# rsutormin/KmerGutsJava

Hardware: AMD Instinct MI355X
Metric: amino-acid residues/sec scanned (and hits/sec) on 1 Gbp synthetic, 1/2/4/8 MI355X (higher is better)
Workload: dtype int64; 1 GPU; 1 Gbp contig mix (0.5 kbp..1.024 Mbp, uniform ACGT) on 1 GPU, 6-frame translate + 8-mer lookup vs 1400303159-slot signature table (33.6 GB, load 0.50), -m 5 -g 200; total_bp_rank0=1000000000, contigs_rank0=6351, total_bp_all_ranks=1000000000, num_sigs=1400303159, residues_rank0=1999974596, residues_all_ranks=1999974596, hits_rank0=36744843, hits_all_ranks=36744843, calls_rank0=4, parallelism=contig shards x1, table replicated

## Files before the change

kmergutsjava_amd/csrc/kg_host_plan.hpp:

```cpp
#pragma once

namespace {


template <typename T, T V, T... Vs, typename F>
void dispatch(T x, F &&f)
{
    if constexpr (sizeof...(Vs) == 0) f(std::integral_constant<T, V>{});
    else if (x == V) f(std::integral_constant<T, V>{});
    else dispatch<T, Vs...>(x, f);
}

struct BatchPlan {
    std::vector<uint32_t> ibase;
    uint64_t nblocks = 0, windows = 0, residues = 0;
    uint64_t n_rows = 0, n_cont = 0;
    int64_t longest = 0;
};

template <bool AA>
int plan_batch(const int64_t *offsets, int64_t n_seqs, BatchPlan &b)
{
    constexpr uint32_t PER = AA ? 1 : 6;
    b.ibase.resize((size_t)n_seqs + 1);
    for (int64_t k = 0; k < n_seqs; k++) {
        int64_t L = offsets[k + 1] - offsets[k];
        if (L < 0) return fail(KG_ERR_ARG, "offsets must be non-decreasing");
        b.longest = std::max(b.longest, L);
        if (L > 0xFFFFFFF0ll) return fail(KG_ERR_LIMIT, "a single sequence longer than 2^32-16 characters");
        b.ibase[(size_t)k] = (uint32_t)b.nblocks;
        uint64_t nb;
        if (AA) {
            uint64_t nwin = L >= 9 ? (uint64_t)L - 8 : 0;
            b.windows += nwin;
            b.residues += (uint64_t)L;
            nb = (nwin + kg::kAaWinPerBlock - 1) / kg::kAaWinPerBlock;
        } else {
            uint64_t npos = L >= 24 ? (uint64_t)L - 23 : 0;
            b.windows += 2 * npos;
            for (int f = 0; f < 3; f++)
                if (L - f >= 3) b.residues += 2 * (uint64_t)((L - f) / 3);
            nb = (npos + kg::kDnaPosPerBlock - 1) / kg::kDnaPosPerBlock;
        }
        b.nblocks += nb;
        if (b.nblocks > 0x7FFFFFFFull / PER) return fail(KG_ERR_LIMIT, "batch too large: more than 2^31-1 window rows; split the batch");
    }
    b.ibase[(size_t)n_seqs] = (uint32_t)b.nblocks;
    if (b.windows > 0xFFFFFF00ull) return fail(KG_ERR_LIMIT, "batch too large: more than 2^32-256 windows; split the batch");
    b.n_rows = b.nblocks * PER;
    b.n_cont = (uint64_t)n_seqs * PER;
    return KG_OK;
}

uint64_t bucket_count(uint64_t limit, uint32_t shift) { return (limit + (1ull << shift) - 1) >> shift; }

struct PartPlan {
    bool applicable = false;
    uint32_t shift = 0, buckets = 0;
    uint32_t n_chunks = 0;
    std::vector<uint64_t> clo;
    std::vector<int64_t> cseq;
    uint64_t max_chunk = 0;
    uint32_t n_wg = 0, cap = 0;
    uint64_t n_regions = 0;
    uint32_t ovf_cap = 0;
    uint32_t gshift = 10, groups_stride = 0;
    size_t next_stride = 0;
    size_t scatter_lds = 0;
    bool use_bidx = false, part_counters = false, prog_index = false;
    uint32_t probe_grid = 0, index_grid = 0, verify_grid = 0, lowc_grid = 0, ovf_grid = 0, order_grid = 0;
    uint32_t scatter_prio = 0, index_prio = 0, verify_prio = 0, index_r = 1, probe_grab = 0;
    uint32_t flush_list = 0;
    uint64_t list_slack = 0, ucap = 0, ccap = 0;
    uint32_t n_os = 0;
    bool early_totals = false, place_staged = false, debug = false;
};

template <bool AA>
int plan_partition(const kg_table *t, const BatchPlan &b, bool progress, bool counters_req, PartPlan &pl)
{
    constexpr uint32_t PER = AA ? 1 : 6;
    const uint64_t nblocks = b.nblocks;
    uint32_t shift = env_knob("KG_PART_SHIFT", 21u, 4u, 31u);
    const uint64_t qmax = (uint64_t)KG_MAX_ENCODED / (uint64_t)t->num_sigs + 1;
    while (shift > 4 && qmax >= (1ull << (32 - shift))) shift--;
    while (bucket_count(t->limit, shift) > (uint64_t)kg::kMaxBuckets) shift++;
    while (kg::scatter_lds_bytes<AA>((uint32_t)bucket_count(t->limit, shift)) > 160u * 1024) shift++;
    const bool fits = shift < 32 && qmax < (1ull << (32 - shift)) && nblocks <= (1ull << 23) && t->m35 != 0 &&
                      t->limit < (1ull << 32) - 64;
    const uint32_t mode = env_u32("KG_PARTITION", 2u);
    const bool worth = t->limit >= (64ull << 20) && b.windows >= (1ull << 27);
    if (!(fits && nblocks > 0 && (mode == 1 || (mode == 2 && worth)))) return KG_OK;
    pl.shift = shift;
    pl.buckets = (uint32_t)bucket_count(t->limit, shift);

    constexpr uint32_t WIN = AA ? 64u : 384u;
    uint32_t want = env_u32("KG_PART_CHUNKS", 4u);
    if (want < 1) want = 1;
    if (want > kMaxChunks) want = kMaxChunks;
    if (getenv("KG_PART_MIN_CHUNK_BLOCKS")) {
        const uint64_t min_chunk = std::max(1u, env_u32("KG_PART_MIN_CHUNK_BLOCKS", 600000u));
        while (want > 1 && nblocks / want < min_chunk) want--;
    } else {
        const uint32_t by_size = nblocks < 450000 ? 1u : std::max(2u, (uint32_t)std::lround(std::sqrt((double)nblocks / 325000.0)));
        want = std::min(want, std::max(1u, by_size));
    }
    pl.clo.push_back(0); pl.cseq.push_back(0);
    std::vector<double> cum;
    if (const char *tp = getenv("KG_PART_TAPER")) {
        double acc = 0;
        for (const char *q = tp; *q;) {
            char *endp = nullptr;
            const double v = strtod(q, &endp);
            if (endp == q) break;
            acc += v; cum.push_back(acc);
            q = *endp == ',' ? endp + 1 : endp;
        }
        if (cum.size() >= 2 && cum.size() <= kMaxChunks && acc > 0) { for (auto &x : cum) x /= acc; want = (uint32_t)cum.size(); }
        else cum.clear();
    }
    for (uint32_t c = 1; c < want; c++) {
        const uint64_t target = cum.empty() ? nblocks * c / want : (uint64_t)((double)nblocks * cum[c - 1]);
        const auto it = std::lower_bound(b.ibase.begin(), b.ibase.end(), (uint32_t)target);
        const uint64_t cut = *it;
        if (cut > pl.clo.back() && cut < nblocks) { pl.clo.push_back(cut); pl.cseq.push_back((int64_t)(it - b.ibase.begin())); }
    }
    pl.clo.push_back(nblocks); pl.cseq.push_back((int64_t)b.ibase.size() - 1);
    pl.n_chunks = (uint32_t)pl.clo.size() - 1;
    for (uint32_t c = 0; c < pl.n_chunks; c++) pl.max_chunk = std::max(pl.max_chunk, pl.clo[c + 1] - pl.clo[c]);
    const uint64_t max_chunk = pl.max_chunk;
    const uint64_t chunk_blocks = (max_chunk + kg::kScatterWaves - 1) / kg::kScatterWaves * kg::kScatterWaves;
    const double max_frac = (double)max_chunk / (double)nblocks;
    uint32_t n_wg = env_knob("KG_PART_WGS", 256u, 1u, kMaxGrid);
    if ((uint64_t)n_wg * kg::kScatterWaves > chunk_blocks) n_wg = (uint32_t)((chunk_blocks + kg::kScatterWaves - 1) / kg::kScatterWaves);
    const uint64_t blocks_per_wg = ((chunk_blocks + (uint64_t)n_wg * kg::kScatterWaves - 1) / ((uint64_t)n_wg * kg::kScatterWaves)) * kg::kScatterWaves;
    const double mean = (double)blocks_per_wg * WIN / (double)pl.buckets * (env_u32("KG_PART_SLACK", 100u) / 100.0);
    const uint64_t cap64 = ((uint64_t)(mean + 6.0 * std::sqrt(mean) + 32.0) + 15) / 16 * 16;
    if (cap64 >= (1ull << 24) || (uint64_t)pl.buckets * n_wg >= (1ull << 24)) return KG_OK;
    pl.n_wg = n_wg;
    pl.cap = (uint32_t)cap64;
    pl.n_regions = (uint64_t)pl.buckets * n_wg;
    pl.ovf_cap = env_u32("KG_PART_OVF_GROUPS", (uint32_t)std::min<uint64_t>(1u << 23, std::max<uint64_t>(65536, pl.n_regions * pl.cap / 16 / 8)));
    while (pl.gshift < 12 && ((max_chunk * PER) >> pl.gshift) + 2 > 8192) pl.gshift++;
    pl.groups_stride = (uint32_t)(((max_chunk * PER) >> pl.gshift) + 2);
    if (pl.groups_stride > kg::kMaxGroups) return fail(KG_ERR_LIMIT, "a chunk of the batch holds more than 2^26 window rows");
    pl.next_stride = std::max<size_t>((size_t)pl.buckets + 8, 256);
    pl.use_bidx = t->d_bidx != nullptr && !counters_req && env_u32("KG_BIDX", 1u) != 0;
    pl.part_counters = (counters_req || progress) && !pl.use_bidx;
    pl.prog_index = progress && pl.use_bidx;
    pl.scatter_lds = kg::scatter_lds_bytes<AA>(pl.buckets);
    pl.flush_list = env_knob("KG_SCATTER_FLUSH_LIST", kg::scatter_flush_list_max<AA>(), 1u, kg::scatter_flush_list_max<AA>());
    pl.probe_grid = env_knob("KG_PROBE_GRID", 256u * 8u, 8u, kMaxGrid, 8u);
    pl.index_grid = env_knob("KG_INDEX_GRID", 256u * 4u, 8u, kMaxGrid, 8u);
    pl.scatter_prio = std::min(3u, env_u32("KG_SCATTER_PRIO", 1u));
    pl.index_prio = std::min(3u, env_u32("KG_INDEX_PRIO", 2u));
    pl.verify_prio = std::min(3u, env_u32("KG_VERIFY_PRIO", pl.n_chunks == 1 ? 2u : 0u));
    uint32_t index_r = env_u32("KG_INDEX_R", 0u);
    if (index_r == 0) index_r = mean * 0.7 >= 640.0 ? 1u : mean * 0.7 >= 320.0 ? 2u : 4u;
    if (index_r != 1 && index_r != 2) index_r = 4;
    while (index_r > 1 && (n_wg % index_r != 0 || kg::kIndexN % index_r != 0)) index_r /= 2;
    pl.index_r = index_r;
    pl.verify_grid = env_knob("KG_VERIFY_GRID", 256u * 2u, 1u, kMaxGrid);
    pl.lowc_grid = env_knob("KG_LOWC_GRID", 256u, 1u, kMaxGrid);
    pl.ovf_grid = env_knob("KG_OVF_GRID", 256u, 1u, kMaxGrid);
    pl.list_slack = (uint64_t)(std::max(std::max(pl.probe_grid, pl.index_grid), pl.verify_grid) + 64) * 4 * kg::kUChunk + 4096;
    pl.ucap = ((uint64_t)((double)b.windows * t->stage_ratio * max_frac) + pl.list_slack + kg::kUChunk - 1) / kg::kUChunk * kg::kUChunk;
    pl.ccap = ((uint64_t)((double)b.windows * (t->stage_ratio * 1.25 + 0.03) * max_frac) + pl.list_slack + kg::kUChunk - 1) /
              kg::kUChunk * kg::kUChunk;
    if (test_hook("KG_TEST_TINY_LISTS")) pl.ucap = pl.ccap = kg::kUChunk;
    const uint32_t grab_unit = 256u * (uint32_t)std::max(kg::kProbeN, kg::kIndexN);
    pl.probe_grab = env_knob("KG_PROBE_GRAB", pl.cap, grab_unit, 1u << 24, grab_unit);
    pl.n_os = pl.n_chunks < 2 ? 0u : std::min(env_u32("KG_ORDER_STREAMS", 0u), kMaxOrderStreams);
    pl.early_totals = pl.n_os == 0 && env_u32("KG_EARLY_TOTALS", 1u) != 0;
    pl.order_grid = env_knob("KG_ORDER_GRID", 256u * 3u, 1u, kMaxGrid);
    pl.place_staged = pl.gshift == 10 && env_u32("KG_PLACE_STAGED", 1u) != 0;
    pl.debug = getenv("KG_DEBUG") != nullptr;
    pl.applicable = true;
    return KG_OK;
}

struct DirectPlan {
    uint32_t scan_grid, stage_chunk;
    const uint32_t *d_hbits;
    uint32_t rpg;
    uint64_t stage_cap;
};

template <bool AA>
DirectPlan plan_direct(const kg_table *t, const BatchPlan &b, bool counters)
{
    DirectPlan pl;
    pl.scan_grid = env_knob("KG_SCAN_GRID", 256u * 8u, 1u, kMaxGrid);
    pl.stage_chunk = env_knob("KG_STAGE_CHUNK", 256u, 1u, 1u << 12);
    const uint32_t filter_mode = env_u32("KG_DIRECT_FILTER", 1u);
    pl.d_hbits = (counters || filter_mode == 0 || (filter_mode == 1 && t->limit <= (4ull << 20))) ? nullptr : t->d_hbits;
    pl.rpg = AA ? 1u : env_u32("KG_SCAN_RPG", pl.d_hbits ? 6u : 3u);
    if (pl.rpg != 1 && pl.rpg != 2 && pl.rpg != 3 && pl.rpg != 6) pl.rpg = 3;
    pl.stage_cap = (uint64_t)((double)b.windows * t->stage_ratio) + 4096 + (uint64_t)pl.scan_grid * kg::kWavesPerWG * pl.stage_chunk;
    if (pl.stage_cap > 0xFFFFFF00ull) pl.stage_cap = 0xFFFFFF00ull;
    if (test_hook("KG_TEST_TINY_LISTS")) pl.stage_cap = 256;
    return pl;
}

struct AggPlan {
    uint32_t pshift;
    bool pieces_on;
    uint32_t agg_pairs;
};

AggPlan plan_aggregate()
{
    AggPlan pl;
    pl.pshift = std::min(20u, std::max(6u, env_u32("KG_AGG_BLOCK_SHIFT", 9u)));
    pl.pieces_on = env_u32("KG_AGG_PIECES", 1u) != 0;
    pl.agg_pairs = env_u32("KG_AGG_PAIRS", 1u);
    return pl;
}

}
```

kmergutsjava_amd/csrc/kg_host_scan.hpp:

```cpp
#pragma once

namespace {

struct ScanCtx {
    kg_table *t;
    kg_result *res;
    Scratch &sc;
    const BatchPlan &b;
    const uint8_t *d_seq, *h_seq;
    const int64_t *offsets;
    int64_t n_seqs;
    bool progress, counters;
    bool seq_uploaded;
    uint64_t n_hits = 0;
    int64_t *d_off = nullptr;
    uint32_t *d_ibase = nullptr;
    kg::BlockDesc *d_blocks = nullptr;
    uint32_t *d_counts = nullptr, *d_offs = nullptr, *d_bsb = nullptr;
    uint64_t *d_partial = nullptr, *d_totals = nullptr;
    kg::Progress *d_prog = nullptr;
};

int upload_seq(const ScanCtx &cx, int64_t a, int64_t b)
{
// ... 220 lines not shown
            hipLaunchKernelGGL((kg::bucket_tag_kernel<COUNTERS>), dim3(pl.probe_grid), dim3(256), 0, s2, t->d_tags, t->limit,
                               (uint64_t)t->num_sigs, v.ent, v.fill, pl.n_wg, pl.cap, pl.buckets, pl.shift, pl.probe_grab, v.next, v.cand,
                               v.candused, v.ccur, pb.ccap, d_ctr, COUNTERS ? d_prog : (kg::Progress *)nullptr);
        });
    }
    HIP_TRY(hipEventRecord(t->pev[kPevChunk + 2 * v.c + 1], s2));
    HIP_TRY(hipStreamWaitEvent(s3, t->pev[kPevChunk + 2 * v.c + 1], 0));
    dispatch<int, 1, 2, 0>(pl.part_counters ? 1 : pl.prog_index ? 2 : 0, [&](auto walks) {
        constexpr bool COUNTERS = decltype(walks)::value == 1, PROG = decltype(walks)::value == 2;
        hipLaunchKernelGGL((kg::verify_kernel<AA, COUNTERS, PROG>), dim3(pl.verify_grid), dim3(256), 0, s3, t->d_entries, t->d_tags, t->limit,
                           (uint64_t)t->num_sigs, t->magic, v.cand, v.candused, v.ccur, pb.ccap, v.ulist, v.cused, v.ucur, pb.ucap, d_ctr,
                           d_prog, pl.verify_prio);
        hipLaunchKernelGGL((kg::overflow_probe_kernel<AA, COUNTERS, PROG>), dim3(pl.ovf_grid), dim3(256), 0, s3, t->d_entries, t->d_tags,
                           t->limit, (uint64_t)t->num_sigs, t->magic, v.ovf_bucket, v.ovf_ent, v.ovfc, pl.ovf_cap, pl.shift, v.ulist,
                           v.cused, v.ucur, pb.ucap, d_ctr, d_prog);
    });
    HIP_TRY(hipEventRecord(t->pev[kPevVerified + v.c], s3));
    HIP_TRY(hipGetLastError());
    return KG_OK;
}

template <bool AA>
int chunk_order(const ScanCtx &cx, const PartPlan &pl, const PartBuffers &pb, const ChunkView &v, uint64_t hits_cap)
{
    constexpr uint32_t PER = AA ? 1 : 6;
    kg_table *t = cx.t;
    kg_result *res = cx.res;
    const uint32_t c = v.c, gshift = pl.gshift;
    const bool last = c + 1 == pl.n_chunks;
    hipStream_t s = t->stream;
    if (pl.n_os) {
        s = t->ostream[c % pl.n_os];
        HIP_TRY(hipStreamWaitEvent(s, t->ev[kEvScattered], 0));
    }
    HIP_TRY(hipStreamWaitEvent(s, t->pev[kPevVerified + c], 0));
    const uint64_t row_lo = (uint64_t)v.lo * PER, row_hi = row_lo + (uint64_t)v.nb * PER;
    const uint32_t g0 = (uint32_t)(row_lo >> gshift);
    const uint32_t n_groups = v.nb ? (uint32_t)(((row_hi - 1) >> gshift) - g0 + 1) : 1u;
    hipLaunchKernelGGL(kg::hit_hist_kernel, dim3(pl.order_grid), dim3(kg::kHThreads), (size_t)n_groups * 4, s, v.ulist, v.cused, v.ucur, pb.ucap,
                       g0, 6u + gshift, n_groups, v.ghist);
    hipLaunchKernelGGL(kg::group_scan_kernel, dim3(1), dim3(kg::kGsThreads), 0, s, v.ghist, n_groups, v.gbase, v.gcur1, v.gcur2, v.ctot, v.gtile);
    if (pl.n_os && c) HIP_TRY(hipStreamWaitEvent(s, t->pev[kPevBase + c - 1], 0));
    hipLaunchKernelGGL(kg::chunk_base_kernel, dim3(1), dim3(1), 0, s, v.ctot, v.base, last ? cx.d_totals : (uint64_t *)nullptr);
    if (pl.n_os) HIP_TRY(hipEventRecord(t->pev[kPevBase + c], s));
    if (pl.early_totals && last) {
        int rc;
        if ((rc = send_counters(t, pb.d_pc, pb.d_ovfc, cx.d_totals, s))) return rc;
        HIP_TRY(hipEventRecord(t->pev[kPevTotals], s));
    }
    hipLaunchKernelGGL((kg::hit_partition_kernel<true>), dim3(pl.order_grid), dim3(kg::kHThreads), 0, s, v.ulist, v.cused, v.ucur, pb.ucap,
                       v.gbase, n_groups, g0, 6u + gshift, v.gcur1, v.sortA, pb.ucap, v.gtile);
    hipLaunchKernelGGL((kg::hit_partition_kernel<false>), dim3(pl.order_grid), dim3(kg::kHThreads), 0, s, v.sortA, v.cused, v.ucur, pb.ucap,
                       v.gbase, n_groups, g0, 6u + gshift, v.gcur2, v.sortB, pb.ucap, v.gtile);
    hipLaunchKernelGGL((kg::group_place_kernel<AA>), dim3(std::min(n_groups, 256u * 8u)), dim3(kg::kHThreads),
                       kg::group_place_lds(gshift, pl.place_staged), s,
                       v.sortB, v.gbase, n_groups, g0, gshift, (uint32_t)row_lo, (uint32_t)row_hi, pb.d_geo, (uint64_t)cx.b.n_rows,
                       pl.place_staged ? 1u : 0u, v.base, res->d_hits, hits_cap, cx.d_offs, res->d_hit_slots);
    HIP_TRY(hipGetLastError());
    return KG_OK;
}

template <bool AA>
int part_allocate(ScanCtx &cx, const PartPlan &pl, PartBuffers &pb)
{
    kg_table *t = cx.t;
    Scratch &sc = cx.sc;
    const uint32_t n_chunks = pl.n_chunks, groups_stride = pl.groups_stride;
    int rc;
    if ((rc = sc.get(&pb.d_ent, (size_t)(pl.n_regions * pl.cap * n_chunks)))) return rc;
    if ((rc = sc.get(&pb.d_fill, (size_t)pl.n_regions * n_chunks))) return rc;
    if ((rc = sc.get(&pb.d_ovf_ent, (size_t)pl.ovf_cap * kg::kGroup * n_chunks))) return rc;
    if ((rc = sc.get(&pb.d_ovf_bucket, (size_t)pl.ovf_cap * n_chunks))) return rc;
    if ((rc = sc.get(&pb.d_next, pl.next_stride * n_chunks))) return rc;
    if ((rc = sc.get(&pb.d_ovfc, kOvfWords * kMaxChunks))) return rc;
    if ((rc = sc.get(&pb.d_lowc, (size_t)cx.b.nblocks + 1))) return rc;
    if ((rc = sc.get(&pb.d_geo, (size_t)cx.b.n_rows))) return rc;
    if ((rc = sc.get(&pb.d_ghist, (size_t)groups_stride * n_chunks))) return rc;
    if ((rc = sc.get(&pb.d_gbase, (size_t)(groups_stride + 1) * n_chunks))) return rc;
    if ((rc = sc.get(&pb.d_gcur1, (size_t)(kg::kHDigits + 1) * n_chunks))) return rc;
    if ((rc = sc.get(&pb.d_gcur2, (size_t)groups_stride * n_chunks))) return rc;
    if ((rc = sc.get(&pb.d_gtile, (size_t)(kg::kHDigits + 1) * n_chunks))) return rc;
    if (kg::group_place_lds(pl.gshift, pl.gshift == 10) > t->place_lds[AA ? 1 : 0]) {
        const size_t want_lds = kg::group_place_lds(pl.gshift, pl.gshift == 10);
        HIP_TRY(hipFuncSetAttribute((const void *)kg::group_place_kernel<AA>, hipFuncAttributeMaxDynamicSharedMemorySize, (int)want_lds));
        t->place_lds[AA ? 1 : 0] = want_lds;
    }
    if (groups_stride * 4u > t->hist_lds) {
        HIP_TRY(hipFuncSetAttribute((const void *)kg::hit_hist_kernel, hipFuncAttributeMaxDynamicSharedMemorySize, (int)(groups_stride * 4u)));
        t->hist_lds = groups_stride * 4u;
    }
    if ((rc = sc.get(&pb.d_pc, kPcWords))) return rc;
    const int sv = scatter_variant_of(cx);
    if (t->scatter_lds[AA ? 1 : 0][sv] < pl.scatter_lds) {
        hipError_t e = hipSuccess;
        scatter_variant(sv, [&](auto is_short, auto prog) {
            e = hipFuncSetAttribute((const void *)kg::part_scatter_kernel<AA, decltype(is_short)::value, decltype(prog)::value>,
                                    hipFuncAttributeMaxDynamicSharedMemorySize, (int)pl.scatter_lds);
        });
        HIP_TRY(e);
        t->scatter_lds[AA ? 1 : 0][sv] = pl.scatter_lds;
    }
    return KG_OK;
}

template <bool AA>
int scan_partitioned(ScanCtx &cx, const PartPlan &pl, bool &done)
{
    constexpr uint32_t PER = AA ? 1 : 6;
    kg_table *t = cx.t;
    kg_result *res = cx.res;
    kg_stats &st = res->st;
    const uint32_t n_chunks = pl.n_chunks;
    const uint64_t nblocks = cx.b.nblocks;
    int rc;
    PartBuffers pb;
    if ((rc = part_allocate<AA>(cx, pl, pb))) return rc;
    BlockGuard<6> lists{cx.sc, {(void **)&pb.d_ulist, (void **)&pb.d_cused, (void **)&pb.d_cand, (void **)&pb.d_candused,
                                (void **)&pb.d_sortA, (void **)&pb.d_sortB}};
    pb.ucap = pl.ucap; pb.ccap = pl.ccap;
    HIP_TRY(hipEventRecord(t->ev[kEvScanBegin], t->stream));
    for (int attempt = 0; attempt < 3; attempt++) {
        const uint64_t ucap = pb.ucap, ccap = pb.ccap;
        const uint64_t hits_cap = ucap * n_chunks;
        pb.cused_stride = (size_t)(ucap / kg::kUChunk + 1); pb.candused_stride = (size_t)(ccap / kg::kUChunk + 1);
        if ((rc = dalloc(t, (void **)&res->d_hits, hits_cap * sizeof(kg_hit)))) return rc;
        if (cx.progress && (rc = dalloc(t, (void **)&res->d_hit_slots, hits_cap * 4))) return rc;
        if ((rc = dalloc(t, (void **)&pb.d_ulist, ucap * n_chunks * sizeof(kg_hit)))) return rc;
        if ((rc = dalloc(t, (void **)&pb.d_cused, pb.cused_stride * n_chunks * 4))) return rc;
        if ((rc = dalloc(t, (void **)&pb.d_cand, ccap * n_chunks * sizeof(kg::CandRec)))) return rc;
        if ((rc = dalloc(t, (void **)&pb.d_candused, pb.candused_stride * n_chunks * 4))) return rc;
        if ((rc = dalloc(t, (void **)&pb.d_sortA, ucap * n_chunks * sizeof(kg_hit)))) return rc;
        if ((rc = dalloc(t, (void **)&pb.d_sortB, ucap * n_chunks * sizeof(kg_hit)))) return rc;
        if ((rc = clear_words(t->stream, [](uint64_t most) { return (uint32_t)std::min<uint64_t>(4096, (most / 4 + 255) / 256 + 1); },
                              {{pb.d_cused, (uint64_t)pb.cused_stride * n_chunks},
                               {pb.d_candused, (uint64_t)pb.candused_stride * n_chunks},
                               {pb.d_pc, kPcWords * 2},
                               {cx.d_totals, kTotWords * 2},
// ... 270 lines not shown
```

kmergutsjava_amd/csrc/kg_order.hpp:

```cpp
#pragma once

#include "kg_device.hpp"
#include "kg_partition.hpp"

namespace kg {

constexpr uint32_t kHThreads = 512;
constexpr uint32_t kHPer = 4;
constexpr uint32_t kHTile = kHThreads * kHPer;
constexpr uint32_t kHDigits = 128;
constexpr uint32_t kMaxGroups = kHDigits * kHDigits;

struct RowGeo { uint32_t container; int32_t pos_first; };

template <bool AA>
__global__ void row_geo_kernel(const BlockDesc *__restrict__ blocks, uint32_t n_blocks, RowGeo *__restrict__ geo)
{
    constexpr uint32_t ROWS = AA ? 1 : 6;
    const uint64_t tl = (uint64_t)blockIdx.x * blockDim.x + threadIdx.x;
    if (tl >= (uint64_t)n_blocks * ROWS) return;
    const uint32_t r = (uint32_t)(tl / n_blocks), it = (uint32_t)(tl % n_blocks);
    const BlockDesc bd = blocks[it];
    RowGeo g;
    int32_t pos0;
// ... 44 lines not shown
        }
        uint32_t incl = mine;
        for (int off = 1; off < 64; off <<= 1) {
            const uint32_t y = __shfl_up(incl, off);
            if (lane >= off) incl += y;
        }
        if (lane == 63) wsum[wave] = incl;
        __syncthreads();
        uint32_t wbase = 0, all = 0;
        for (int w = 0; w < (int)(kGsThreads / 64); w++) {
            const uint32_t sw = wsum[w];
            if (w < wave) wbase += sw;
            all += sw;
        }
        const uint32_t c = carry;
        uint32_t e = c + wbase + incl - mine;
#pragma unroll
        for (uint32_t k = 0; k < kGsPer; k++) {
            const uint32_t i = i0 + k;
            if (i < n_groups) {
                gbase[i] = e;
                cur2[i] = e;
                if ((i & (kHDigits - 1)) == 0) cur1[i / kHDigits] = e;
            }
            e += x[k];
        }
        __syncthreads();
        if (threadIdx.x == 0) carry = c + all;
        __syncthreads();
    }
    const uint32_t n_d1 = (n_groups + kHDigits - 1) / kHDigits;
    if (threadIdx.x == 0) {
        gbase[n_groups] = carry;
        cur1[n_d1] = carry;
        *total_out = carry;
    }
    __syncthreads();
    const uint32_t d = threadIdx.x;
    const uint32_t t = d < n_d1 ? (cur1[d + 1] - cur1[d] + kHTile - 1) / kHTile : 0u;
    uint32_t incl = t;
    for (int off = 1; off < 64; off <<= 1) {
        const uint32_t y = __shfl_up(incl, off);
        if (lane >= off) incl += y;
    }
    if (d == 63) wsum[0] = incl;
    __syncthreads();
    if (d < kHDigits) {
        const uint32_t before = d >= 64 ? wsum[0] : 0u;
        tile_start[d] = before + incl - t;
        if (d == kHDigits - 1) tile_start[kHDigits] = before + incl;
    }
}

template <bool FIRST>
__global__ __launch_bounds__(kHThreads) void hit_partition_kernel(const kg_hit *__restrict__ in, const uint32_t *__restrict__ chunk_used,
                                                                  const unsigned long long *__restrict__ cursor, uint64_t in_cap,
                                                                  const uint32_t *__restrict__ gbase, uint32_t n_groups, uint32_t g0, uint32_t gs,
                                                                  uint32_t *cur, kg_hit *__restrict__ out, uint64_t out_cap,
                                                                  const uint32_t *__restrict__ tile_start)
{
    __shared__ __attribute__((aligned(16))) kg_hit stage[kHTile];
    __shared__ uint32_t hist[kHDigits], cnt[kHDigits], sbase[kHDigits], gb[kHDigits];
    const uint32_t tid = threadIdx.x, lane = tid & 63u, wave = tid >> 6;
    if (tid < kHDigits) hist[tid] = 0;
    const uint32_t n_d1 = (n_groups + kHDigits - 1) / kHDigits;
    uint32_t n_res = 0;
    if (FIRST) {
        const unsigned long long cc = *cursor;
        n_res = (uint32_t)((cc < in_cap ? cc : in_cap) / kUChunk);
    }
    __shared__ uint32_t tstart[kHDigits + 1];
    if (!FIRST) {
        if (tid <= kHDigits) tstart[tid] = tile_start[tid];
        __syncthreads();
    }
    const uint32_t n_items = FIRST ? (n_res + kHTile / kUChunk - 1) / (kHTile / kUChunk) : tstart[kHDigits];
    {
        for (uint32_t item = blockIdx.x; item < n_items; item += gridDim.x) {
            uint32_t d1 = 0, tile = item;
            if (!FIRST) {
                uint32_t lo_d = 0, hi_d = n_d1;
                while (hi_d - lo_d > 1) {
                    const uint32_t mid = (lo_d + hi_d) / 2;
                    if (tstart[mid] <= item) lo_d = mid; else hi_d = mid;
                }
                d1 = lo_d;
                tile = item - tstart[d1];
            }
            const uint32_t seg_lo = FIRST ? 0u : gbase[d1 * kHDigits];
            const uint32_t seg_hi = FIRST ? 0u : gbase[min((d1 + 1) * kHDigits, n_groups)];
            kg_hit rec[kHPer];
            uint32_t dr[kHPer];
#pragma unroll
            for (uint32_t k = 0; k < kHPer; k++) {
                const uint32_t i = k * kHThreads + tid;
                bool ok;
                uint64_t at;
                if (FIRST) {
                    const uint32_t c = tile * (kHTile / kUChunk) + i / kUChunk;
                    ok = c < n_res && (i % kUChunk) < chunk_used[c];
                    at = (uint64_t)c * kUChunk + (i % kUChunk);
                } else {
                    at = (uint64_t)seg_lo + (uint64_t)tile * kHTile + i;
                    ok = at < seg_hi;
                }
                dr[k] = ~0u;
                if (ok) {
                    rec[k] = stream_load_hit(in + at);
                    const uint32_t g = (rec[k].container >> gs) - g0;
                    if (g < n_groups) {
                        const uint32_t d = FIRST ? g / kHDigits : g % kHDigits;
                        dr[k] = (d << 16) | atomicAdd(&hist[d], 1u);
                    }
                }
            }
            __syncthreads();
            if (tid < kHDigits) {
                const uint32_t c = hist[tid];
                uint32_t incl = c;
                for (int off = 1; off < 64; off <<= 1) {
                    const uint32_t y = __shfl_up(incl, off);
                    if ((int)lane >= off) incl += y;
                }
                cnt[tid] = c;
                sbase[tid] = incl - c;
                gb[tid] = c ? atomicAdd(&cur[FIRST ? tid : d1 * kHDigits + tid], c) : 0u;
                hist[tid] = 0;
            }
            __syncthreads();
            const uint32_t first_half = sbase[63] + cnt[63];
#pragma unroll
            for (uint32_t k = 0; k < kHPer; k++)
                if (dr[k] != ~0u) {
                    const uint32_t d = dr[k] >> 16;
                    stage[sbase[d] + (d >= 64 ? first_half : 0u) + (dr[k] & 0xFFFFu)] = rec[k];
                }
            __syncthreads();
            const uint64_t *stage64 = reinterpret_cast<const uint64_t *>(stage);
            uint64_t *out64 = reinterpret_cast<uint64_t *>(out);
            for (uint32_t d = wave; d < kHDigits; d += kHThreads / 64u) {
                const uint32_t n = cnt[d];
                if (n == 0) continue;
                const uint32_t s0 = sbase[d] + (d >= 64 ? first_half : 0u);
                const uint64_t o0 = gb[d];
                const uint32_t n_ok = o0 >= out_cap ? 0u : (uint32_t)min((uint64_t)n, out_cap - o0);
                for (uint32_t i = lane; i < 3u * n_ok; i += 64u) stream_store8(out64 + o0 * 3u + i, stage64[(uint64_t)s0 * 3u + i]);
            }
            __syncthreads();
        }
    }
}

constexpr uint32_t kPlaceOut = 1536;
__host__ __device__ inline size_t group_place_lds(uint32_t gshift, bool staged)
{
    return staged ? ((size_t)20 << gshift) + (size_t)kPlaceOut * sizeof(kg_hit) : ((size_t)12 << gshift);
}
template <bool AA>
__global__ __launch_bounds__(kHThreads) void group_place_kernel(const kg_hit *__restrict__ in, const uint32_t *__restrict__ gbase, uint32_t n_groups,
                                                                uint32_t g0, uint32_t gshift, uint32_t row_lo, uint32_t row_hi ,
                                                                const RowGeo *__restrict__ geo, uint64_t n_rows_all, uint32_t staged,
                                                                const uint64_t *__restrict__ base,
                                                                kg_hit *__restrict__ hits, uint64_t hits_cap, uint32_t *__restrict__ offs,
                                                                uint32_t *__restrict__ hit_slots )
{
    extern __shared__ __attribute__((aligned(16))) unsigned char p_lds[];
    const uint32_t R = 1u << gshift;
    unsigned long long *masks = reinterpret_cast<unsigned long long *>(p_lds);
    uint32_t *pre = reinterpret_cast<uint32_t *>(masks + R);
    RowGeo *lgeo = reinterpret_cast<RowGeo *>(pre + R);
    uint64_t *lout = reinterpret_cast<uint64_t *>(lgeo + R);
    __shared__ uint32_t wsum[kHThreads / 64];
    const uint32_t tid = threadIdx.x, lane = tid & 63u, wave = tid >> 6;
    const uint64_t chunk_base = *base;
    const uint32_t per = R / kHThreads > 0 ? R / kHThreads : 1u;
    for (uint32_t g = blockIdx.x; g < n_groups; g += gridDim.x) {
        const uint32_t lo = gbase[g], n = gbase[g + 1] - lo;
        const uint64_t row0 = (uint64_t)(g0 + g) << gshift;
        const bool to_lds = staged && n <= kPlaceOut;
        for (uint32_t i = tid; i < R; i += kHThreads) {
            masks[i] = 0ull;
            if (staged && n && row0 + i < n_rows_all) lgeo[i] = geo[row0 + i];
        }
        __syncthreads();
        constexpr uint32_t kKeep = 4;
        const bool keep = n <= kHThreads * kKeep;
        kg_hit rk[kKeep];
        if (keep) {
#pragma unroll
            for (uint32_t j = 0; j < kKeep; j++) {
                const uint32_t k = j * kHThreads + tid;
                if (k < n) {
                    rk[j] = stream_load_hit(in + lo + k);
                    atomicOr(&masks[(rk[j].container >> 6) & (R - 1u)], 1ull << (rk[j].container & 63u));
                }
            }
        } else {
            for (uint32_t k = tid; k < n; k += kHThreads) {
                const uint32_t key = in[lo + k].container;
                atomicOr(&masks[(key >> 6) & (R - 1u)], 1ull << (key & 63u));
            }
        }
        __syncthreads();
        uint32_t mine = 0;
        const uint32_t r_lo = tid * per;
        if (r_lo < R)
            for (uint32_t i = 0; i < per; i++) mine += (uint32_t)__popcll(masks[r_lo + i]);
        uint32_t incl = mine;
        for (int off = 1; off < 64; off <<= 1) {
            const uint32_t y = __shfl_up(incl, off);
            if ((int)lane >= off) incl += y;
        }
        if (lane == 63) wsum[wave] = incl;
        __syncthreads();
        uint32_t run = incl - mine;
        for (uint32_t w = 0; w < wave; w++) run += wsum[w];
        if (r_lo < R)
            for (uint32_t i = 0; i < per; i++) {
                pre[r_lo + i] = run;
                const uint64_t row = row0 + r_lo + i;
                if (row >= row_lo && row < row_hi) offs[row] = (uint32_t)(chunk_base + lo + run);
                run += (uint32_t)__popcll(masks[r_lo + i]);
            }
        __syncthreads();
        auto place = [&](kg_hit h) {
            const uint32_t key = h.container, rl = (key >> 6) & (R - 1u), ol = key & 63u;
            const RowGeo gr = staged ? lgeo[rl] : geo[key >> 6];
            const uint32_t rank = pre[rl] + (uint32_t)__popcll(masks[rl] & ((1ull << ol) - 1ull));
            if (hit_slots && chunk_base + lo + rank < hits_cap)
                hit_slots[chunk_base + lo + rank] = (uint32_t)h.from0InProt;
            h.container = gr.container;
            h.from0InProt = gr.pos_first + (int32_t)ol;
            if (to_lds) {
                uint64_t w3[3];
                __builtin_memcpy(w3, &h, 24);
                lout[3u * rank] = w3[0]; lout[3u * rank + 1] = w3[1]; lout[3u * rank + 2] = w3[2];
            } else {
                const uint64_t dst = chunk_base + lo + rank;
                if (dst < hits_cap) hits[dst] = h;
            }
        };
        if (keep) {
#pragma unroll
            for (uint32_t j = 0; j < kKeep; j++)
                if (j * kHThreads + tid < n) place(rk[j]);
        } else {
            for (uint32_t k = tid; k < n; k += kHThreads) place(in[lo + k]);
        }
        __syncthreads();
        if (to_lds) {
            const uint64_t dst0 = chunk_base + lo;
            const uint32_t n_ok = dst0 >= hits_cap ? 0u : (uint32_t)min((uint64_t)n, hits_cap - dst0);
            uint64_t *out64 = reinterpret_cast<uint64_t *>(hits) + dst0 * 3u;
            for (uint32_t i = tid; i < 3u * n_ok; i += kHThreads) stream_store8(out64 + i, lout[i]);
            __syncthreads();
        }
    }
}

__global__ __launch_bounds__(256) void restore_hits_kernel(const kg_hit *__restrict__ src, uint64_t n_hits, const int64_t *__restrict__ seq_first,
                                                           uint64_t n_seqs, const int64_t *__restrict__ dst_first,
                                                           const int32_t *__restrict__ container_shift, kg_hit *__restrict__ dst)
{
    __shared__ uint64_t k_first;
    constexpr uint64_t kTile = 1024;
    const uint64_t n_tiles = (n_hits + kTile - 1) / kTile;
    for (uint64_t tile = blockIdx.x; tile < n_tiles; tile += gridDim.x) {
        __syncthreads();
        if (threadIdx.x == 0) {
            const uint64_t i0 = tile * kTile;
            uint64_t lo = 0, hi = n_seqs;
            while (hi - lo > 1) {
                const uint64_t mid = lo + (hi - lo) / 2;
                if ((uint64_t)seq_first[mid] <= i0) lo = mid; else hi = mid;
            }
            k_first = lo;
        }
        __syncthreads();
        uint64_t k = k_first;
#pragma unroll
        for (int j = 0; j < 4; j++) {
            const uint64_t i = tile * kTile + (uint64_t)j * 256 + threadIdx.x;
            if (i < n_hits) {
                while (k + 1 < n_seqs && (uint64_t)seq_first[k + 1] <= i) k++;
                kg_hit h = src[i];
                h.container += (uint32_t)container_shift[k];
                dst[(uint64_t)dst_first[k] + (i - (uint64_t)seq_first[k])] = h;
            }
        }
    }
}

}
```

Before: 133.1 billion residues/s.

## Software-pipeline hit partition and group place kernels with next-tile prefetch

The hit partition kernel is restructured so each block loads its next tile of hits into registers while the current tile is being scattered to the staging buffer. The group place kernel likewise prefetches the next group's row geometry and hits during ranking and placement, and the staged path is specialised at compile time into its own kernel with a waves-per-EU hint. A separate grid-size knob is also added for the place kernel. The aim is to hide global load latency in the hit-ordering stage, at the cost of more register pressure and a more complex loop structure.

```diff
diff --git a/kmergutsjava_amd/csrc/kg_host_plan.hpp b/kmergutsjava_amd/csrc/kg_host_plan.hpp
--- a/kmergutsjava_amd/csrc/kg_host_plan.hpp
+++ b/kmergutsjava_amd/csrc/kg_host_plan.hpp
@@ -68,13 +68,15 @@
     size_t next_stride = 0;
     size_t scatter_lds = 0;
     bool use_bidx = false, part_counters = false, prog_index = false;
-    uint32_t probe_grid = 0, index_grid = 0, verify_grid = 0, lowc_grid = 0, ovf_grid = 0, order_grid = 0;
+    uint32_t probe_grid = 0, index_grid = 0, verify_grid = 0, lowc_grid = 0, ovf_grid = 0, order_grid = 0, place_grid = 0;
     uint32_t scatter_prio = 0, index_prio = 0, verify_prio = 0, index_r = 1, probe_grab = 0;
     uint32_t flush_list = 0;
     uint64_t list_slack = 0, ucap = 0, ccap = 0;
     uint32_t n_os = 0;
     bool early_totals = false, place_staged = false, debug = false;
 };
+
+constexpr uint32_t kPlaceGridDefault = 256u * 8u;
 
 template <bool AA>
 int plan_partition(const kg_table *t, const BatchPlan &b, bool progress, bool counters_req, PartPlan &pl)
@@ -173,7 +175,9 @@
     pl.n_os = pl.n_chunks < 2 ? 0u : std::min(env_u32("KG_ORDER_STREAMS", 0u), kMaxOrderStreams);
     pl.early_totals = pl.n_os == 0 && env_u32("KG_EARLY_TOTALS", 1u) != 0;
     pl.order_grid = env_knob("KG_ORDER_GRID", 256u * 3u, 1u, kMaxGrid);
-    pl.place_staged = pl.gshift == 10 && env_u32("KG_PLACE_STAGED", 1u) != 0;
+    const char *og = getenv("KG_ORDER_GRID");
+    pl.place_grid = env_knob("KG_PLACE_GRID", og && *og ? pl.order_grid : kPlaceGridDefault, 1u, kMaxGrid);
+    pl.place_staged = pl.gshift == kg::kStagedShift && env_u32("KG_PLACE_STAGED", 1u) != 0;
     pl.debug = getenv("KG_DEBUG") != nullptr;
     pl.applicable = true;
     return KG_OK;
diff --git a/kmergutsjava_amd/csrc/kg_host_scan.hpp b/kmergutsjava_amd/csrc/kg_host_scan.hpp
--- a/kmergutsjava_amd/csrc/kg_host_scan.hpp
+++ b/kmergutsjava_amd/csrc/kg_host_scan.hpp
@@ -296,10 +296,15 @@
                        v.gbase, n_groups, g0, 6u + gshift, v.gcur1, v.sortA, pb.ucap, v.gtile);
     hipLaunchKernelGGL((kg::hit_partition_kernel<false>), dim3(pl.order_grid), dim3(kg::kHThreads), 0, s, v.sortA, v.cused, v.ucur, pb.ucap,
                        v.gbase, n_groups, g0, 6u + gshift, v.gcur2, v.sortB, pb.ucap, v.gtile);
-    hipLaunchKernelGGL((kg::group_place_kernel<AA>), dim3(std::min(n_groups, 256u * 8u)), dim3(kg::kHThreads),
-                       kg::group_place_lds(gshift, pl.place_staged), s,
-                       v.sortB, v.gbase, n_groups, g0, gshift, (uint32_t)row_lo, (uint32_t)row_hi, pb.d_geo, (uint64_t)cx.b.n_rows,
-                       pl.place_staged ? 1u : 0u, v.base, res->d_hits, hits_cap, cx.d_offs, res->d_hit_slots);
+    const dim3 place_grid(std::min(n_groups, pl.place_grid));
+    if (pl.place_staged)
+        hipLaunchKernelGGL((kg::group_place_kernel<AA>), place_grid, dim3(kg::kHThreads), kg::group_place_lds(gshift, true), s,
+                           v.sortB, v.gbase, n_groups, g0, (uint32_t)row_lo, (uint32_t)row_hi, pb.d_geo, (uint64_t)cx.b.n_rows,
+                           v.base, res->d_hits, hits_cap, cx.d_offs, res->d_hit_slots);
+    else
+        hipLaunchKernelGGL((kg::group_place_direct_kernel<AA>), place_grid, dim3(kg::kHThreads), kg::group_place_lds(gshift, false), s,
+                           v.sortB, v.gbase, n_groups, g0, gshift, (uint32_t)row_lo, (uint32_t)row_hi, pb.d_geo, (uint64_t)cx.b.n_rows,
+                           v.base, res->d_hits, hits_cap, cx.d_offs, res->d_hit_slots);
     HIP_TRY(hipGetLastError());
     return KG_OK;
 }
@@ -324,9 +329,10 @@
     if ((rc = sc.get(&pb.d_gcur1, (size_t)(kg::kHDigits + 1) * n_chunks))) return rc;
     if ((rc = sc.get(&pb.d_gcur2, (size_t)groups_stride * n_chunks))) return rc;
     if ((rc = sc.get(&pb.d_gtile, (size_t)(kg::kHDigits + 1) * n_chunks))) return rc;
-    if (kg::group_place_lds(pl.gshift, pl.gshift == 10) > t->place_lds[AA ? 1 : 0]) {
-        const size_t want_lds = kg::group_place_lds(pl.gshift, pl.gshift == 10);
+    if (kg::group_place_lds(pl.gshift, pl.gshift == kg::kStagedShift) > t->place_lds[AA ? 1 : 0]) {
+        const size_t want_lds = kg::group_place_lds(pl.gshift, pl.gshift == kg::kStagedShift);
         HIP_TRY(hipFuncSetAttribute((const void *)kg::group_place_kernel<AA>, hipFuncAttributeMaxDynamicSharedMemorySize, (int)want_lds));
+        HIP_TRY(hipFuncSetAttribute((const void *)kg::group_place_direct_kernel<AA>, hipFuncAttributeMaxDynamicSharedMemorySize, (int)want_lds));
         t->place_lds[AA ? 1 : 0] = want_lds;
     }
     if (groups_stride * 4u > t->hist_lds) {
diff --git a/kmergutsjava_amd/csrc/kg_order.hpp b/kmergutsjava_amd/csrc/kg_order.hpp
--- a/kmergutsjava_amd/csrc/kg_order.hpp
+++ b/kmergutsjava_amd/csrc/kg_order.hpp
@@ -120,6 +120,8 @@
     }
 }
 
+static_assert(kUChunk == kHThreads && kHTile / kUChunk == kHPer, "slot k of thread tid = slot tid of the tile's k-th reservation chunk");
+struct PartTile { uint32_t d1, tile, seg_lo, seg_hi, used[kHPer]; };
 template <bool FIRST>
 __global__ __launch_bounds__(kHThreads) void hit_partition_kernel(const kg_hit *__restrict__ in, const uint32_t *__restrict__ chunk_used,
                                                                   const unsigned long long *__restrict__ cursor, uint64_t in_cap,
@@ -138,101 +140,130 @@
         n_res = (uint32_t)((cc < in_cap ? cc : in_cap) / kUChunk);
     }
     __shared__ uint32_t tstart[kHDigits + 1];
-    if (!FIRST) {
-        if (tid <= kHDigits) tstart[tid] = tile_start[tid];
-        __syncthreads();
-    }
+    if (!FIRST && tid <= kHDigits) tstart[tid] = tile_start[tid];
+    __syncthreads();
     const uint32_t n_items = FIRST ? (n_res + kHTile / kUChunk - 1) / (kHTile / kUChunk) : tstart[kHDigits];
-    {
-        for (uint32_t item = blockIdx.x; item < n_items; item += gridDim.x) {
-            uint32_t d1 = 0, tile = item;
-            if (!FIRST) {
-                uint32_t lo_d = 0, hi_d = n_d1;
-                while (hi_d - lo_d > 1) {
-                    const uint32_t mid = (lo_d + hi_d) / 2;
-                    if (tstart[mid] <= item) lo_d = mid; else hi_d = mid;
+    auto tile_of = [&](uint32_t item) {
+        PartTile t = {};
+        t.tile = item;
+        if (FIRST) {
+#pragma unroll
+            for (uint32_t k = 0; k < kHPer; k++) {
+                const uint32_t c = item * kHPer + k;
+                t.used[k] = c < n_res ? chunk_used[c] : 0u;
+            }
+        } else {
+            uint32_t lo_d = 0, hi_d = n_d1;
+            while (hi_d - lo_d > 1) {
+                const uint32_t mid = (lo_d + hi_d) / 2;
+                if (tstart[mid] <= item) lo_d = mid; else hi_d = mid;
+            }
+            t.d1 = lo_d;
+            t.tile = item - tstart[lo_d];
+            t.seg_lo = gbase[lo_d * kHDigits];
+            t.seg_hi = gbase[min((lo_d + 1) * kHDigits, n_groups)];
+        }
+        return t;
+    };
+    auto request = [&](const PartTile &t, kg_hit (&rec)[kHPer]) {
+        uint32_t okm = 0;
+#pragma unroll
+        for (uint32_t k = 0; k < kHPer; k++) {
+            bool ok;
+            uint64_t at;
+            if (FIRST) {
+                ok = tid < t.used[k];
+                at = (uint64_t)(t.tile * kHPer + k) * kUChunk + tid;
+            } else {
+                at = (uint64_t)t.seg_lo + (uint64_t)t.tile * kHTile + k * kHThreads + tid;
+                ok = at < t.seg_hi;
+            }
+            if (ok) {
+                rec[k] = stream_load_hit(in + at);
+                okm |= 1u << k;
+            }
+        }
+        return okm;
+    };
+    uint32_t item = blockIdx.x;
+    if (item >= n_items) return;
+    kg_hit rec[kHPer];
+    PartTile t = tile_of(item);
+    uint32_t okm = request(t, rec);
+    for (;;) {
+        const uint32_t item_next = item + gridDim.x;
+        const bool more = item_next < n_items;
+        PartTile t_next = {};
+        if (more) t_next = tile_of(item_next);
+        uint32_t dr[kHPer];
+#pragma unroll
+        for (uint32_t k = 0; k < kHPer; k++) {
+            dr[k] = ~0u;
+            if (okm >> k & 1u) {
+                const uint32_t g = (rec[k].container >> gs) - g0;
+                if (g < n_groups) {
+                    const uint32_t d = FIRST ? g / kHDigits : g % kHDigits;
+                    dr[k] = (d << 16) | atomicAdd(&hist[d], 1u);
                 }
-                d1 = lo_d;
-                tile = item - tstart[d1];
-            }
-            const uint32_t seg_lo = FIRST ? 0u : gbase[d1 * kHDigits];
-            const uint32_t seg_hi = FIRST ? 0u : gbase[min((d1 + 1) * kHDigits, n_groups)];
-            kg_hit rec[kHPer];
-            uint32_t dr[kHPer];
-#pragma unroll
-            for (uint32_t k = 0; k < kHPer; k++) {
-                const uint32_t i = k * kHThreads + tid;
-                bool ok;
-                uint64_t at;
-                if (FIRST) {
-                    const uint32_t c = tile * (kHTile / kUChunk) + i / kUChunk;
-                    ok = c < n_res && (i % kUChunk) < chunk_used[c];
-                    at = (uint64_t)c * kUChunk + (i % kUChunk);
-                } else {
-                    at = (uint64_t)seg_lo + (uint64_t)tile * kHTile + i;
-                    ok = at < seg_hi;
-                }
-                dr[k] = ~0u;
-                if (ok) {
-                    rec[k] = stream_load_hit(in + at);
-                    const uint32_t g = (rec[k].container >> gs) - g0;
-                    if (g < n_groups) {
-                        const uint32_t d = FIRST ? g / kHDigits : g % kHDigits;
-                        dr[k] = (d << 16) | atomicAdd(&hist[d], 1u);
-                    }
-                }
-            }
-            __syncthreads();
-            if (tid < kHDigits) {
-                const uint32_t c = hist[tid];
-                uint32_t incl = c;
-                for (int off = 1; off < 64; off <<= 1) {
-                    const uint32_t y = __shfl_up(incl, off);
-                    if ((int)lane >= off) incl += y;
-                }
-                cnt[tid] = c;
-                sbase[tid] = incl - c;
-                gb[tid] = c ? atomicAdd(&cur[FIRST ? tid : d1 * kHDigits + tid], c) : 0u;
-                hist[tid] = 0;
-            }
-            __syncthreads();
-            const uint32_t first_half = sbase[63] + cnt[63];
-#pragma unroll
-            for (uint32_t k = 0; k < kHPer; k++)
-                if (dr[k] != ~0u) {
-                    const uint32_t d = dr[k] >> 16;
-                    stage[sbase[d] + (d >= 64 ? first_half : 0u) + (dr[k] & 0xFFFFu)] = rec[k];
-                }
-            __syncthreads();
-            const uint64_t *stage64 = reinterpret_cast<const uint64_t *>(stage);
-            uint64_t *out64 = reinterpret_cast<uint64_t *>(out);
-            for (uint32_t d = wave; d < kHDigits; d += kHThreads / 64u) {
-                const uint32_t n = cnt[d];
-                if (n == 0) continue;
-                const uint32_t s0 = sbase[d] + (d >= 64 ? first_half : 0u);
-                const uint64_t o0 = gb[d];
-                const uint32_t n_ok = o0 >= out_cap ? 0u : (uint32_t)min((uint64_t)n, out_cap - o0);
-                for (uint32_t i = lane; i < 3u * n_ok; i += 64u) stream_store8(out64 + o0 * 3u + i, stage64[(uint64_t)s0 * 3u + i]);
-            }
-            __syncthreads();
-        }
+            }
+        }
+        __syncthreads();
+        if (tid < kHDigits) {
+            const uint32_t c = hist[tid];
+            uint32_t incl = c;
+            for (int off = 1; off < 64; off <<= 1) {
+                const uint32_t y = __shfl_up(incl, off);
+                if ((int)lane >= off) incl += y;
+            }
+            cnt[tid] = c;
+            sbase[tid] = incl - c;
+            gb[tid] = c ? atomicAdd(&cur[FIRST ? tid : t.d1 * kHDigits + tid], c) : 0u;
+            hist[tid] = 0;
+        }
+        __syncthreads();
+        const uint32_t first_half = sbase[63] + cnt[63];
+#pragma unroll
+        for (uint32_t k = 0; k < kHPer; k++)
+            if (dr[k] != ~0u) {
+                const uint32_t d = dr[k] >> 16;
+                stage[sbase[d] + (d >= 64 ? first_half : 0u) + (dr[k] & 0xFFFFu)] = rec[k];
+            }
+        if (more) okm = request(t_next, rec);
+        __syncthreads();
+        const uint64_t *stage64 = reinterpret_cast<const uint64_t *>(stage);
+        uint64_t *out64 = reinterpret_cast<uint64_t *>(out);
+        for (uint32_t d = wave; d < kHDigits; d += kHThreads / 64u) {
+            const uint32_t n = cnt[d];
+            if (n == 0) continue;
+            const uint32_t s0 = sbase[d] + (d >= 64 ? first_half : 0u);
+            const uint64_t o0 = gb[d];
+            const uint32_t n_ok = o0 >= out_cap ? 0u : (uint32_t)min((uint64_t)n, out_cap - o0);
+            for (uint32_t i = lane; i < 3u * n_ok; i += 64u) stream_store8(out64 + o0 * 3u + i, stage64[(uint64_t)s0 * 3u + i]);
+        }
+        if (!more) break;
+        __syncthreads();
+        item = item_next;
+        t = t_next;
     }
 }
 
 constexpr uint32_t kPlaceOut = 1536;
+constexpr uint32_t kStagedShift = 10;
+constexpr uint32_t kGeoPer = (1u << kStagedShift) / kHThreads;
 __host__ __device__ inline size_t group_place_lds(uint32_t gshift, bool staged)
 {
     return staged ? ((size_t)20 << gshift) + (size_t)kPlaceOut * sizeof(kg_hit) : ((size_t)12 << gshift);
 }
-template <bool AA>
-__global__ __launch_bounds__(kHThreads) void group_place_kernel(const kg_hit *__restrict__ in, const uint32_t *__restrict__ gbase, uint32_t n_groups,
-                                                                uint32_t g0, uint32_t gshift, uint32_t row_lo, uint32_t row_hi ,
-                                                                const RowGeo *__restrict__ geo, uint64_t n_rows_all, uint32_t staged,
-                                                                const uint64_t *__restrict__ base,
-                                                                kg_hit *__restrict__ hits, uint64_t hits_cap, uint32_t *__restrict__ offs,
-                                                                uint32_t *__restrict__ hit_slots )
+template <bool STAGED>
+__device__ __forceinline__ void group_place_body(const kg_hit *__restrict__ in, const uint32_t *__restrict__ gbase, uint32_t n_groups,
+                                                 uint32_t g0, uint32_t gshift_any, uint32_t row_lo, uint32_t row_hi ,
+                                                 const RowGeo *__restrict__ geo, uint64_t n_rows_all, const uint64_t *__restrict__ base,
+                                                 kg_hit *__restrict__ hits, uint64_t hits_cap, uint32_t *__restrict__ offs,
+                                                 uint32_t *__restrict__ hit_slots )
 {
     extern __shared__ __attribute__((aligned(16))) unsigned char p_lds[];
+    constexpr bool staged = STAGED;
+    const uint32_t gshift = STAGED ? kStagedShift : gshift_any;
     const uint32_t R = 1u << gshift;
     unsigned long long *masks = reinterpret_cast<unsigned long long *>(p_lds);
     uint32_t *pre = reinterpret_cast<uint32_t *>(masks + R);
@@ -242,55 +273,68 @@
     const uint32_t tid = threadIdx.x, lane = tid & 63u, wave = tid >> 6;
     const uint64_t chunk_base = *base;
     const uint32_t per = R / kHThreads > 0 ? R / kHThreads : 1u;
-    for (uint32_t g = blockIdx.x; g < n_groups; g += gridDim.x) {
-        const uint32_t lo = gbase[g], n = gbase[g + 1] - lo;
+    constexpr uint32_t kKeep = 4;
+    auto request = [&](uint32_t g, uint32_t lo, uint32_t n, RowGeo (&gr)[kGeoPer], kg_hit (&rk)[kKeep]) {
+        if (staged && n) {
+            const uint64_t row0 = (uint64_t)(g0 + g) << gshift;
+#pragma unroll
+            for (uint32_t j = 0; j < kGeoPer; j++)
+                gr[j] = geo[min(row0 + j * kHThreads + tid, n_rows_all - 1u)];
+        }
+        if (n <= kHThreads * kKeep) {
+#pragma unroll
+            for (uint32_t j = 0; j < kKeep; j++) {
+                const uint32_t k = j * kHThreads + tid;
+                if (k < n) rk[j] = stream_load_hit(in + lo + k);
+            }
+        }
+    };
+    uint32_t g = blockIdx.x;
+    if (g >= n_groups) return;
+    uint32_t lo = gbase[g], n = gbase[g + 1] - lo;
+    RowGeo gr[kGeoPer] = {};
+    kg_hit rk[kKeep] = {};
+    request(g, lo, n, gr, rk);
+    for (;;) {
+        const uint32_t g_next = g + gridDim.x;
+        const bool more = g_next < n_groups;
+        uint32_t lo_next = 0, n_next = 0;
+        if (more) {
+            lo_next = gbase[g_next];
+            n_next = gbase[g_next + 1] - lo_next;
+        }
         const uint64_t row0 = (uint64_t)(g0 + g) << gshift;
         const bool to_lds = staged && n <= kPlaceOut;
-        for (uint32_t i = tid; i < R; i += kHThreads) {
-            masks[i] = 0ull;
-            if (staged && n && row0 + i < n_rows_all) lgeo[i] = geo[row0 + i];
-        }
-        __syncthreads();
-        constexpr uint32_t kKeep = 4;
+        for (uint32_t i = tid; i < R; i += kHThreads) masks[i] = 0ull;
+        if (staged && n) {
+#pragma unroll
+            for (uint32_t j = 0; j < kGeoPer; j++) lgeo[j * kHThreads + tid] = gr[j];
+        }
+        __syncthreads();
         const bool keep = n <= kHThreads * kKeep;
-        kg_hit rk[kKeep];
-        if (keep) {
-#pragma unroll
-            for (uint32_t j = 0; j < kKeep; j++) {
-                const uint32_t k = j * kHThreads + tid;
-                if (k < n) {
-                    rk[j] = stream_load_hit(in + lo + k);
-                    atomicOr(&masks[(rk[j].container >> 6) & (R - 1u)], 1ull << (rk[j].container & 63u));
+        auto rank_rows = [&]() {
+            uint32_t mine = 0;
+            const uint32_t r_lo = tid * per;
+            if (r_lo < R)
+                for (uint32_t i = 0; i < per; i++) mine += (uint32_t)__popcll(masks[r_lo + i]);
+            uint32_t incl = mine;
+            for (int off = 1; off < 64; off <<= 1) {
+                const uint32_t y = __shfl_up(incl, off);
+                if ((int)lane >= off) incl += y;
+            }
+            if (lane == 63) wsum[wave] = incl;
+            __syncthreads();
+            uint32_t run = incl - mine;
+            for (uint32_t w = 0; w < wave; w++) run += wsum[w];
+            if (r_lo < R)
+                for (uint32_t i = 0; i < per; i++) {
+                    pre[r_lo + i] = run;
+                    const uint64_t row = row0 + r_lo + i;
+                    if (row >= row_lo && row < row_hi) offs[row] = (uint32_t)(chunk_base + lo + run);
+                    run += (uint32_t)__popcll(masks[r_lo + i]);
                 }
-            }
-        } else {
-            for (uint32_t k = tid; k < n; k += kHThreads) {
-                const uint32_t key = in[lo + k].container;
-                atomicOr(&masks[(key >> 6) & (R - 1u)], 1ull << (key & 63u));
-            }
-        }
-        __syncthreads();
-        uint32_t mine = 0;
-        const uint32_t r_lo = tid * per;
-        if (r_lo < R)
-            for (uint32_t i = 0; i < per; i++) mine += (uint32_t)__popcll(masks[r_lo + i]);
-        uint32_t incl = mine;
-        for (int off = 1; off < 64; off <<= 1) {
-            const uint32_t y = __shfl_up(incl, off);
-            if ((int)lane >= off) incl += y;
-        }
-        if (lane == 63) wsum[wave] = incl;
-        __syncthreads();
-        uint32_t run = incl - mine;
-        for (uint32_t w = 0; w < wave; w++) run += wsum[w];
-        if (r_lo < R)
-            for (uint32_t i = 0; i < per; i++) {
-                pre[r_lo + i] = run;
-                const uint64_t row = row0 + r_lo + i;
-                if (row >= row_lo && row < row_hi) offs[row] = (uint32_t)(chunk_base + lo + run);
-                run += (uint32_t)__popcll(masks[r_lo + i]);
-            }
-        __syncthreads();
+            __syncthreads();
+        };
         auto place = [&](kg_hit h) {
             const uint32_t key = h.container, rl = (key >> 6) & (R - 1u), ol = key & 63u;
             const RowGeo gr = staged ? lgeo[rl] : geo[key >> 6];
@@ -311,9 +355,25 @@
         if (keep) {
 #pragma unroll
             for (uint32_t j = 0; j < kKeep; j++)
+                if (j * kHThreads + tid < n) atomicOr(&masks[(rk[j].container >> 6) & (R - 1u)], 1ull << (rk[j].container & 63u));
+            __syncthreads();
+        } else {
+            for (uint32_t k = tid; k < n; k += kHThreads) {
+                const uint32_t key = in[lo + k].container;
+                atomicOr(&masks[(key >> 6) & (R - 1u)], 1ull << (key & 63u));
+            }
+            __syncthreads();
+            rank_rows();
+            for (uint32_t k = tid; k < n; k += kHThreads) place(in[lo + k]);
+        }
+        RowGeo gr_next[kGeoPer] = {};
+        kg_hit rk_next[kKeep] = {};
+        if (more) request(g_next, lo_next, n_next, gr_next, rk_next);
+        if (keep) {
+            rank_rows();
+#pragma unroll
+            for (uint32_t j = 0; j < kKeep; j++)
                 if (j * kHThreads + tid < n) place(rk[j]);
-        } else {
-            for (uint32_t k = tid; k < n; k += kHThreads) place(in[lo + k]);
         }
         __syncthreads();
         if (to_lds) {
@@ -323,7 +383,34 @@
             for (uint32_t i = tid; i < 3u * n_ok; i += kHThreads) stream_store8(out64 + i, lout[i]);
             __syncthreads();
         }
-    }
+        if (!more) break;
+        g = g_next; lo = lo_next; n = n_next;
+#pragma unroll
+        for (uint32_t j = 0; j < kGeoPer; j++) gr[j] = gr_next[j];
+#pragma unroll
+        for (uint32_t j = 0; j < kKeep; j++) rk[j] = rk_next[j];
+    }
+}
+#define KG_PLACE_REGS __attribute__((amdgpu_waves_per_eu(5)))
+template <bool AA>
+__global__ __launch_bounds__(kHThreads) KG_PLACE_REGS void group_place_kernel(const kg_hit *__restrict__ in, const uint32_t *__restrict__ gbase, uint32_t n_groups,
+                                                                              uint32_t g0, uint32_t row_lo, uint32_t row_hi,
+                                                                              const RowGeo *__restrict__ geo, uint64_t n_rows_all,
+                                                                              const uint64_t *__restrict__ base, kg_hit *__restrict__ hits,
+                                                                              uint64_t hits_cap, uint32_t *__restrict__ offs,
+                                                                              uint32_t *__restrict__ hit_slots)
+{
+    group_place_body<true>(in, gbase, n_groups, g0, kStagedShift, row_lo, row_hi, geo, n_rows_all, base, hits, hits_cap, offs, hit_slots);
+}
+template <bool AA>
+__global__ __launch_bounds__(kHThreads) KG_PLACE_REGS void group_place_direct_kernel(const kg_hit *__restrict__ in, const uint32_t *__restrict__ gbase,
+                                                                                     uint32_t n_groups, uint32_t g0, uint32_t gshift, uint32_t row_lo,
+                                                                                     uint32_t row_hi, const RowGeo *__restrict__ geo, uint64_t n_rows_all,
+                                                                                     const uint64_t *__restrict__ base, kg_hit *__restrict__ hits,
+                                                                                     uint64_t hits_cap, uint32_t *__restrict__ offs,
+                                                                                     uint32_t *__restrict__ hit_slots)
+{
+    group_place_body<false>(in, gbase, n_groups, g0, gshift, row_lo, row_hi, geo, n_rows_all, base, hits, hits_cap, offs, hit_slots);
 }
 
 __global__ __launch_bounds__(256) void restore_hits_kernel(const kg_hit *__restrict__ src, uint64_t n_hits, const int64_t *__restrict__ seq_first,
```

Result: no change. 133.3 billion residues/s (median of 2 runs) (+0.2%).
